# Alxaline/BraTS21

Hardware: AMD Instinct MI355X
Metric: train patches/sec (4x128^3, width-48) (higher is better)
Workload: dtype bf16; 1 GPU; equiunet width=48, batch=2/GPU of 4x128^3 synthetic patches, fwd + deep-supervision Dice + bwd + ranger (BASELINE.json configs[1]); global_batch=2, parallelism=dp1

## Files before the change

### brats21_amd/csrc/dice.hip

```cpp
#include "common.hpp"

__global__ void dice_stats_kernel(const float* __restrict__ x, const float* __restrict__ t, float* __restrict__ part, int K,
                                  size_t voxels) {
  const int nk = blockIdx.y, k = nk % K;
  const float* xp = x + (size_t)nk * voxels;
  const float* tp = t + (size_t)nk * voxels;
  float s0 = 0.f, s1 = 0.f, s2 = 0.f;
  const size_t v4 = (voxels % 4 == 0 && (((size_t)x | (size_t)t) & 15) == 0) ? voxels / 4 : 0;
  for (size_t i = (size_t)blockIdx.x * blockDim.x + threadIdx.x; i < v4; i += (size_t)gridDim.x * blockDim.x) {
    const f32x4 xv = ((const f32x4*)xp)[i], tv = ((const f32x4*)tp)[i];
#pragma unroll
    for (int j = 0; j < 4; ++j) {
      const float p = 1.f / (1.f + __expf(-xv[j]));
      s0 += tv[j] * p;
      s1 += p * p;
      s2 += tv[j] * tv[j];
    }
  }
  for (size_t i = v4 * 4 + (size_t)blockIdx.x * blockDim.x + threadIdx.x; i < voxels; i += (size_t)gridDim.x * blockDim.x) {
    const float p = 1.f / (1.f + __expf(-xp[i]));
    s0 += tp[i] * p; s1 += p * p; s2 += tp[i] * tp[i];
  }
  __shared__ float r[3][256];
  r[0][threadIdx.x] = s0; r[1][threadIdx.x] = s1; r[2][threadIdx.x] = s2;
  __syncthreads();
  for (int m = 128; m > 0; m >>= 1) {
    if ((int)threadIdx.x < m) {
      r[0][threadIdx.x] += r[0][threadIdx.x + m];
      r[1][threadIdx.x] += r[1][threadIdx.x + m];
      r[2][threadIdx.x] += r[2][threadIdx.x + m];
    }
    __syncthreads();
  }
  if (threadIdx.x < 3) part[(((size_t)(nk / K) * gridDim.x + blockIdx.x) * K + k) * 3 + threadIdx.x] = r[threadIdx.x][0];
}

__global__ void __launch_bounds__(256) ordered_sum_kernel(const float* __restrict__ part, float* __restrict__ out, int nb, int total,
                                                          float* __restrict__ out2 , int n1) {
  const int e = threadIdx.x & 7, g = threadIdx.x >> 3;
  const int i = blockIdx.x * 8 + e;
  float s = 0.f;
  if (i < total) {
    const float* src = part + i;
    int b = g;
    for (; b + 7 * 32 < nb; b += 8 * 32) {
      float v[8];
#pragma unroll
      for (int u = 0; u < 8; ++u) v[u] = src[(size_t)(b + 32 * u) * total];
// ... 23 lines not shown
}

__global__ void dice_grad_kernel(const float* __restrict__ x, const float* __restrict__ t, const float* __restrict__ coef,
                                 float* __restrict__ dx, int K, size_t voxels) {
  const int nk = blockIdx.y, k = nk % K;
  const float a = coef[k * 2], b2 = 2.f * coef[k * 2 + 1];
  const float* xp = x + (size_t)nk * voxels;
  const float* tp = t + (size_t)nk * voxels;
  float* dp = dx + (size_t)nk * voxels;
  const size_t v4 = (voxels % 4 == 0 && (((size_t)x | (size_t)t | (size_t)dx) & 15) == 0) ? voxels / 4 : 0;
  for (size_t i = (size_t)blockIdx.x * blockDim.x + threadIdx.x; i < v4; i += (size_t)gridDim.x * blockDim.x) {
    const f32x4 xv = ((const f32x4*)xp)[i], tv = ((const f32x4*)tp)[i];
    f32x4 o;
#pragma unroll
    for (int j = 0; j < 4; ++j) {
      const float p = 1.f / (1.f + __expf(-xv[j]));
      o[j] = (a * tv[j] + b2 * p) * p * (1.f - p);
    }
    ((f32x4*)dp)[i] = o;
  }
  for (size_t i = v4 * 4 + (size_t)blockIdx.x * blockDim.x + threadIdx.x; i < voxels; i += (size_t)gridDim.x * blockDim.x) {
    const float p = 1.f / (1.f + __expf(-xp[i]));
    dp[i] = (a * tp[i] + b2 * p) * p * (1.f - p);
  }
}

constexpr int DICE_MAX_BLOCKS = 512;
extern "C" size_t brats_dice_ws_floats(int N, int K) { return (size_t)N * DICE_MAX_BLOCKS * K * 3; }

extern "C" int brats_dice_stats(const float* logits, const float* target, float* sums , float* ws, int N, int K,
                                size_t voxels, brats_stream_t s) {
  if (!logits || !target || !sums || !ws || N <= 0 || K <= 0) BRATS_FAIL(BRATS_E_ARG, "dice_stats: bad argument");
  hipStream_t st = (hipStream_t)s;
  size_t gx = (voxels / 4 + 255) / 256 / 4;
  gx = gx < 1 ? 1 : (gx > DICE_MAX_BLOCKS ? DICE_MAX_BLOCKS : gx);
  hipLaunchKernelGGL(dice_stats_kernel, dim3((unsigned)gx, N * K), dim3(256), 0, st, logits, target, ws, K, voxels);
  brats_ordered_sum(ws, sums, N * (int)gx, K * 3, st);
  BRATS_CHECK_LAUNCH();
  return 0;
}

extern "C" int brats_dice_grad(const float* logits, const float* target, const float* coef ,
                               float* dlogits, int N, int K, size_t voxels, brats_stream_t s) {
  if (!logits || !target || !coef || !dlogits) BRATS_FAIL(BRATS_E_ARG, "dice_grad: null pointer");
  size_t gx = (voxels / 4 + 255) / 256 / 4;
  gx = gx < 1 ? 1 : (gx > 2048 ? 2048 : gx);
  hipLaunchKernelGGL(dice_grad_kernel, dim3((unsigned)gx, N * K), dim3(256), 0, (hipStream_t)s, logits, target, coef, dlogits, K, voxels);
  BRATS_CHECK_LAUNCH();
  return 0;
}
```

### brats21_amd/csrc/pool_up.hip

```cpp
#include "twin_begin.hpp"
#include "common.hpp"

constexpr int POOL_MAX_BLOCKS = 8192;

template <typename T>
__global__ void maxpool2_fwd_kernel(const T* __restrict__ x, int xpitch, T* __restrict__ y, int ypitch, int N, int C,
                                    int D, int H, int W, int with_avg, uint8_t* __restrict__ argmax) {
  constexpr int VW = 16 / sizeof(T);
  const int cv = C / VW, Do = D / 2, Ho = H / 2, Wo = W / 2;
  const size_t total = (size_t)N * Do * Ho * Wo * cv;
  for (size_t it = (size_t)blockIdx.x * blockDim.x + threadIdx.x; it < total; it += (size_t)gridDim.x * blockDim.x) {
    const int c0 = (int)(it % cv) * VW;
    size_t v = it / cv;
    const int xo = v % Wo; v /= Wo;
    const int yo = v % Ho; v /= Ho;
    const int zo = v % Do;
    const int n = (int)(v / Do);
    float mx[VW], sm[VW];
    int am[VW];
#pragma unroll
    for (int j = 0; j < VW; ++j) { mx[j] = -INFINITY; sm[j] = 0.f; am[j] = 0; }
#pragma unroll
    for (int k = 0; k < 8; ++k) {
      const int z = 2 * zo + (k >> 2), yy = 2 * yo + ((k >> 1) & 1), xx = 2 * xo + (k & 1);
// ... 360 lines not shown
    } else {
      with_stream16(dtype, big, [&](auto t, auto nt) { go(t, nt, std::false_type{}); });
    }
    BRATS_CHECK_LAUNCH();
    return 0;
  }
  with_storage(dtype, [&](auto t) {
    using T = typename decltype(t)::type;
    hipLaunchKernelGGL(upsample_fwd_kernel<T>, dim3(grid), dim3(256), 0, (hipStream_t)s, (const T*)x, xpitch, (T*)y, ypitch, N, C, D, H, W,
                       scale, sd, sh, sw);
  });
  BRATS_CHECK_LAUNCH();
  return 0;
}

template <typename TI, typename TO, int VW>
__global__ void lerp_adjoint_kernel(const TI* __restrict__ in, int in_pitch, TO* __restrict__ out, int out_pitch,
                                    size_t outer, int Lout , int Lin , size_t inner_vox, int C,
                                    float scale) {
  const int cv = C / VW;
  const size_t total = outer * Lin * inner_vox * cv;
  const float inv = scale > 0.f ? 1.f / scale : 0.f;
  for (size_t it = (size_t)blockIdx.x * blockDim.x + threadIdx.x; it < total; it += (size_t)gridDim.x * blockDim.x) {
    const int c0 = (int)(it % cv) * VW;
    size_t v = it / cv;
    const size_t iv = v % inner_vox; v /= inner_vox;
    const int i = (int)(v % Lin);
    const size_t o = v / Lin;
    int lo = (int)floorf((float)(i - 1) * inv) - 1, hi = (int)ceilf((float)(i + 1) * inv) + 1;
    if (scale <= 0.f) { lo = 0; hi = Lout - 1; }
    lo = lo < 0 ? 0 : lo;
    hi = hi > Lout - 1 ? Lout - 1 : hi;
    float acc[VW];
#pragma unroll
    for (int j = 0; j < VW; ++j) acc[j] = 0.f;
    for (int l = lo; l <= hi; ++l) {
      const Lerp c = lerp_coef(l, Lin, scale);
      float w = 0.f;
      if (c.i0 == i) w += c.w0;
      if (c.i1 == i) w += c.w1;
      if (w != 0.f) {
        float a[VW];
        if constexpr (VW == 1) a[0] = to_f<TI>(in[((o * Lout + l) * inner_vox + iv) * in_pitch + c0]);
        else Vec<TI, VW>::load(in + ((o * Lout + l) * inner_vox + iv) * in_pitch + c0, a);
#pragma unroll
        for (int j = 0; j < VW; ++j) acc[j] += w * a[j];
      }
    }
    if constexpr (VW == 1) out[((o * Lin + i) * inner_vox + iv) * out_pitch + c0] = from_f<TO>(acc[0]);
    else Vec<TO, VW>::store(out + ((o * Lin + i) * inner_vox + iv) * out_pitch + c0, acc);
  }
}

int brats_lerp_adjoint_f32_planes(const float* in, float* out, size_t outer, int Lout, int Lin, size_t inner,
                                  hipStream_t st) {
  const size_t total = outer * Lin * inner;
  if (inner % 4 == 0 && (((size_t)in | (size_t)out) & 15) == 0) {
    hipLaunchKernelGGL((lerp_adjoint_kernel<float, float, 4>), dim3(stream_grid(total / 4, 256, POOL_MAX_BLOCKS)), dim3(256), 0, st, in, 4,
                       out, 4, outer, Lout, Lin, inner / 4, 4, ac_scale(Lin, Lout));
    BRATS_CHECK_LAUNCH();
    return 0;
  }
  hipLaunchKernelGGL((lerp_adjoint_kernel<float, float, 1>), dim3(stream_grid(total, 256, POOL_MAX_BLOCKS)), dim3(256), 0, st, in, 1, out, 1,
// ... 18 lines not shown
  float w = 0.f;
  if (c.i0 == i) w += c.w0;
  if (c.i1 == i) w += c.w1;
  return w;
}

constexpr int UBF_TH = 4, UBF_TW = 8, UBF_FH = 12, UBF_FW = 20, UBF_CS = 48, UBF_CV = UBF_CS / 8, UBF_THREADS = 512, UBF_KC = 3, UBF_MAXP = 2;
static_assert(UBF_FH * UBF_FW * UBF_CV <= UBF_THREADS * UBF_KC, "every column of the fine footprint needs a thread slot");
DEVI void ubf_add(float* acc, float w, const bf16_t* p) {
  float a[8];
  Vec<bf16_t, 8>::load(p, a);
#pragma unroll
  for (int j = 0; j < 8; ++j) acc[j] += w * a[j];
}
struct UbfStep { int l[UBF_MAXP]; float wc[UBF_MAXP], wn[UBF_MAXP]; int np; };
__global__ void __launch_bounds__(UBF_THREADS, 4) upsample2_bwd_fused_kernel(const bf16_t* __restrict__ dy, int dypitch, bf16_t* __restrict__ dx,
                                                                          int dxpitch, int C, int D, int H, int W, int cd, float sd,
                                                                          float sh, float sw) {
  __shared__ __attribute__((aligned(16))) bf16_t slab[UBF_FH * UBF_FW * UBF_CS];
  __shared__ __attribute__((aligned(16))) bf16_t t2s[UBF_TH * UBF_FW * UBF_CS];
  __shared__ float wys[UBF_TH][UBF_FH], wxs[UBF_TW][UBF_FW];
  __shared__ int yrng[UBF_TH][2], xrng[UBF_TW][2];
  const int Do = 2 * D, Ho = 2 * H, Wo = 2 * W;
  const int nsl = C / UBF_CS, tiles_x = W / UBF_TW, tiles_y = H / UBF_TH, nz = D / cd;
  int bid = blockIdx.x;
  if (gridDim.x % 8 == 0) bid = (bid % 8) * (gridDim.x / 8) + bid / 8;
  const int sl = bid % nsl, tx = (bid / nsl) % tiles_x, ty = (bid / (nsl * tiles_x)) % tiles_y;
  const int zc = (bid / (nsl * tiles_x * tiles_y)) % nz, n = bid / (nsl * tiles_x * tiles_y * nz);
  const int za = zc * cd, ya = ty * UBF_TH, xa = tx * UBF_TW;
  const int tid = threadIdx.x;
  int yl, yh, xl, xh;
  lerp_fine_range(ya, UBF_TH, H, Ho, sh, yl, yh);
  lerp_fine_range(xa, UBF_TW, W, Wo, sw, xl, xh);
// ... 123 lines not shown
        const float w = wys[h][f];
        if (w != 0.f) ubf_add(acc, w, slab + ((size_t)f * rowv + r) * 8);
      }
      Vec<bf16_t, 8>::store(t2s + (size_t)it * 8, acc);
    }
    __syncthreads();
    for (int it = tid; it < UBF_TH * UBF_TW * UBF_CV; it += UBF_THREADS) {
      const int cvi = it % UBF_CV, xc = (it / UBF_CV) % UBF_TW, h = it / (UBF_CV * UBF_TW);
      float acc[8];
#pragma unroll
      for (int j = 0; j < 8; ++j) acc[j] = 0.f;
      for (int f = xrng[xc][0]; f <= xrng[xc][1]; ++f) {
        const float w = wxs[xc][f];
        if (w != 0.f) ubf_add(acc, w, t2s + ((size_t)(h * fw + f) * UBF_CV + cvi) * 8);
      }
      Vec<bf16_t, 8>::store(dst + (((size_t)i * H + ya + h) * W + xa + xc) * dxpitch + cvi * 8, acc);
    }
  }
}

static int g_upsample_bwd_fused = -1;
extern "C" int BRATS_API(brats_upsample_bwd_set_fused)(int mode) {
  const int old = g_upsample_bwd_fused;
  g_upsample_bwd_fused = mode < 0 ? -1 : (mode ? 1 : 0);
  return old;
}
static int upsample_bwd_fused_cd(int N, int C, int D, int H, int W, int sc) {
  if (g_upsample_bwd_fused == 0 || sc != 2 || C % UBF_CS || H % UBF_TH || W % UBF_TW || D % 4) return 0;
  const size_t per_z = (size_t)N * (H / UBF_TH) * (W / UBF_TW) * (C / UBF_CS);
  int cd = 16;
// ... 124 lines not shown
  else PAF_LAUNCH(6, 2);
#undef PAF_LAUNCH
  BRATS_CHECK_LAUNCH();
  return 0;
}

extern "C" size_t BRATS_API(brats_upsample_bwd_ws_bytes)(int dtype, int N, int C, int D, int H, int W, int scale) {
  const size_t esz = dtype == BRATS_BF16 ? 2 : 4;
  const size_t a = (size_t)N * D * (H * scale) * (W * scale) * C;
  const size_t b = (size_t)N * D * H * (W * scale) * C;
  return ((a * esz + 255) / 256 * 256) + ((b * esz + 255) / 256 * 256);
}

template <typename T>
static int upsample_bwd_t(const T* dy, int dypitch, T* dx, int dxpitch, char* tmp, int N, int C, int D, int H, int W, int sc,
                          hipStream_t st) {
  constexpr int VW = 16 / sizeof(T);
  const int Do = D * sc, Ho = H * sc, Wo = W * sc;
  if constexpr (sizeof(T) == 2) {
    if (const int cd = upsample_bwd_fused_cd(N, C, D, H, W, sc)) {
      const dim3 grid((unsigned)((size_t)N * (H / UBF_TH) * (W / UBF_TW) * (C / UBF_CS) * (D / cd)));
      hipLaunchKernelGGL(upsample2_bwd_fused_kernel, grid, dim3(UBF_THREADS), 0, st, dy, dypitch, dx, dxpitch, C, D, H, W, cd,
                         ac_scale(D, Do), ac_scale(H, Ho), ac_scale(W, Wo));
      BRATS_CHECK_LAUNCH();
      return 0;
    }
  }
  const size_t a_elems = (size_t)N * D * Ho * Wo * C;
  T* t1 = (T*)tmp;
  T* t2 = (T*)(tmp + ((a_elems * sizeof(T) + 255) / 256 * 256));
  size_t total = (size_t)N * D * Ho * Wo * (C / VW);
  hipLaunchKernelGGL((lerp_adjoint_kernel<T, T, VW>), dim3(stream_grid(total, 256, POOL_MAX_BLOCKS)), dim3(256), 0, st, dy, dypitch, t1, C,
                     (size_t)N, Do, D, (size_t)Ho * Wo, C, ac_scale(D, Do));
  total = (size_t)N * D * H * Wo * (C / VW);
  hipLaunchKernelGGL((lerp_adjoint_kernel<T, T, VW>), dim3(stream_grid(total, 256, POOL_MAX_BLOCKS)), dim3(256), 0, st, (const T*)t1, C, t2, C,
                     (size_t)N * D, Ho, H, (size_t)Wo, C, ac_scale(H, Ho));
  total = (size_t)N * D * H * W * (C / VW);
  hipLaunchKernelGGL((lerp_adjoint_kernel<T, T, VW>), dim3(stream_grid(total, 256, POOL_MAX_BLOCKS)), dim3(256), 0, st, (const T*)t2, C, dx,
                     dxpitch, (size_t)N * D * H, Wo, W, (size_t)1, C, ac_scale(W, Wo));
  BRATS_CHECK_LAUNCH();
  return 0;
}

extern "C" int BRATS_API(brats_upsample_bwd)(const void* dy, int dypitch, void* dx, int dxpitch, void* tmp, int dtype, int N, int C,
                                  int D, int H, int W, int scale, brats_stream_t s) {
  const int vw = vec_width(dtype);
  if (!dy || !dx || !tmp || C % vw || dypitch % vw || dxpitch % vw) BRATS_FAIL(BRATS_E_ARG, "upsample_bwd: bad argument");
  return with_storage(dtype, [&](auto t) {
    using T = typename decltype(t)::type;
    return upsample_bwd_t<T>((const T*)dy, dypitch, (T*)dx, dxpitch, (char*)tmp, N, C, D, H, W, scale, (hipStream_t)s);
  });
}
#include "twin_end.hpp"
```

### brats21_amd/engine.py

```python
import torch

from . import ops
from .evaluate import Evaluator
from .optim import clip_grad_norm_
from .losses import DiceLoss, deep_supervision_loss, deep_supervision_prepared_loss, fused_deep_supervision_dice


class TrainStep:

    def __init__(self, model, optimizer, criterion=None, amp=True, buckets=None, fused_dice=True, jaccard=False,
                 max_grad_norm=None, amp_dtype=torch.bfloat16, scaler=None):
        self.model, self.optimizer, self.amp, self.buckets = model, optimizer, amp, buckets
        self.fused, self.jaccard, self.max_grad_norm = fused_dice and criterion is None, jaccard, max_grad_norm
        self.criterion = criterion if criterion is not None else DiceLoss(jaccard=jaccard)
        self.amp_dtype = amp_dtype
        self.scaler = scaler
        self._params = None
        if amp and amp_dtype == torch.float16 and scaler is None:
            self.scaler = torch.amp.GradScaler("cuda")

    def loss(self, outputs, target):
        if self.fused:
            return fused_deep_supervision_dice(outputs, target, jaccard=self.jaccard)
        if hasattr(self.criterion, "prepare"):
            return deep_supervision_prepared_loss(self.criterion, outputs, target)[0]
        return deep_supervision_loss(self.criterion, outputs, target)[0]

    def _zero_grad(self):
        params = self._params
        if params is None:
            params = self._params = list(self.model.parameters())
        for p in params:
# ... 2 lines not shown
    def __call__(self, image, target):
        self._zero_grad()
        with torch.autocast("cuda", dtype=self.amp_dtype, enabled=self.amp):
            outputs = self.model(image)
            loss = self.loss(outputs, target)
        if self.scaler is not None and self.amp:
            self.scaler.scale(loss).backward()
            if self.buckets is not None:
                self.buckets.finish()
            if self.max_grad_norm is not None:
                self.scaler.unscale_(self.optimizer)
                clip_grad_norm_(self._params, self.max_grad_norm)
            self.scaler.step(self.optimizer)
            self.scaler.update()
            return loss
        loss.backward()
        if self.buckets is not None:
            self.buckets.finish()
        if self.max_grad_norm is not None:
            clip_grad_norm_(self._params, self.max_grad_norm)
        self.optimizer.step()
        return loss


class GraphedTrainStep:

    def __init__(self, step, warmup=2, multi_rank_capture=None):
        if getattr(step, "scaler", None) is not None and step.amp:
            if not (getattr(step.optimizer, "_step_supports_amp_scaling", False) and getattr(step.optimizer, "capturable", False)):
                raise NotImplementedError("GraphedTrainStep: a TrainStep with a GradScaler (amp_dtype=torch.float16) captures only with "
                                          "an optimizer that implements the GradScaler protocol on the device "
# ... 55 lines not shown
```

### brats21_amd/losses.py

```python
from collections.abc import Sequence

import torch
import torch.nn as nn


class DiceLoss(nn.Module):
    def __init__(self, jaccard=False, smooth_nr=1e-5, smooth_dr=1e-5):
        super().__init__()
        self.jaccard, self.smooth_nr, self.smooth_dr = jaccard, smooth_nr, smooth_dr

    def forward(self, logits, target):
        p = torch.sigmoid(logits.float())
        t = target.float()
        axes = (0, 2, 3, 4)
        inter = (t * p).sum(axes)
        denom = (t * t).sum(axes) + (p * p).sum(axes)
        if self.jaccard:
            denom = 2.0 * (denom - inter)
        return (1.0 - (2.0 * inter + self.smooth_nr) / (denom + self.smooth_dr)).mean()


def flatten_heads(outputs):
    if isinstance(outputs, (tuple, list)):
        return [h for o in outputs for h in flatten_heads(o)]
    return [outputs]


def deep_supervision_loss(criterion, outputs, target):
    if isinstance(outputs, (tuple, list)):
        heads = flatten_heads(outputs)
        return torch.stack([criterion(h, target) for h in heads]).mean(), heads[0]
    return criterion(outputs, target), outputs


class _FusedDiceFn(torch.autograd.Function):

    @staticmethod
    def forward(ctx, target, jaccard, eps, *heads):
        from . import _lib
        lib = _lib.lib()
        st = torch.cuda.current_stream().cuda_stream
        t = target.contiguous().float()
        n, k = t.shape[:2]
        vox = t[0, 0].numel()
        hs = [h.contiguous().float() for h in heads]
        sums = torch.empty((len(hs), k, 3), dtype=torch.float32, device=t.device)
        ws = torch.empty(lib.brats_dice_ws_floats(n, k), dtype=torch.float32, device=t.device)
        for i, h in enumerate(hs):
            _lib.check(lib.brats_dice_stats(h.data_ptr(), t.data_ptr(), sums[i].data_ptr(), ws.data_ptr(), n, k, vox, st), "dice_stats")
        inter, p2, t2 = sums[..., 0], sums[..., 1], sums[..., 2]
        hk = float(len(hs) * k)
        if jaccard:
            den = 2.0 * (t2 + p2 - inter)
            f = 1.0 - (2.0 * inter + eps) / (den + eps)
            dden = (2.0 * inter + eps) / (den + eps) ** 2
            coef = torch.stack([(-2.0 / (den + eps) - 2.0 * dden) / hk, 2.0 * dden / hk], -1)
        else:
            den = t2 + p2
            f = 1.0 - (2.0 * inter + eps) / (den + eps)
            coef = torch.stack([-2.0 / (den + eps) / hk, (2.0 * inter + eps) / (den + eps) ** 2 / hk], -1)
        ctx.save_for_backward(t, coef.contiguous(), *hs)
        return f.mean()

    @staticmethod
    def backward(ctx, g):
        from . import _lib
        lib = _lib.lib()
        st = torch.cuda.current_stream().cuda_stream
        t, coef, *hs = ctx.saved_tensors
        n, k = t.shape[:2]
        vox = t[0, 0].numel()
        coef = (coef * g).contiguous()
        outs = []
        for i, h in enumerate(hs):
            d = torch.empty_like(h)
            _lib.check(lib.brats_dice_grad(h.data_ptr(), t.data_ptr(), coef[i].data_ptr(), d.data_ptr(), n, k, vox, st), "dice_grad")
            outs.append(d)
        return (None, None, None) + tuple(outs)


def fused_deep_supervision_dice(outputs, target, jaccard=False, eps=1e-5):
    heads = flatten_heads(outputs)
    return _FusedDiceFn.apply(target, jaccard, eps, *heads)


def _check_reference_options(name, sigmoid, softmax, to_onehot_y, other_act, reduction):
# ... 393 lines not shown
```

### brats21_amd/networks/equiunet.py

```python
import contextlib
import functools
import math
import os

import torch
import torch.nn as nn

from .. import ops
from .._lib import PACK_DGRAD, PACK_FWD, BratsHipError
from ._program import _PackedWeightsModule, _fn_backward, _fn_forward, _heads_bwd, _inherit_amax, input_cpad


class _ConvParams(nn.Module):

    def __init__(self, cin, cout, k, bias):
        super().__init__()
        self.weight = nn.Parameter(torch.empty(cout, cin, k, k, k))
        self.bias = nn.Parameter(torch.empty(cout)) if bias else None
        nn.init.kaiming_uniform_(self.weight, a=math.sqrt(5))
        if bias:
            bound = 1.0 / math.sqrt(cin * k * k * k)
            nn.init.uniform_(self.bias, -bound, bound)


# ... 422 lines not shown


def _decoder_bwd(ctx, cx, douts):
    m = cx.m
    _, _, _, _, bottom, bottom_2, up3, up2, up1 = ctx.bufs
    cbw = functools.partial(_cgr_bwd, cx)
    c1, c2 = _blk(m.decoder1)
    top, dsrc = _heads_bwd(ctx, cx, douts, m.fold_head_bwd and cx.drop is None and not c2.batch_norm
                           and ops.head_fold_ok(m.outconv.weight, *_unit_act(c2, cx.act)))

    def extra(t):
        return dsrc.get(t.data_ptr())

    d_c1 = cbw(c2, None, head=top, bst=c1) if top is not None else cbw(c2, extra(up1) if extra(up1) is not None else torch.zeros_like(up1), bst=c1)
    d_skip1, d_u1 = cbw(c1, d_c1)
    d_up2 = _plus(ops.upsample_bwd(d_u1, 2), extra(up2))
    c1, c2 = _blk(m.decoder2)
    d_skip2, d_u2 = cbw(c1, cbw(c2, d_up2, bst=c1))
    d_up3 = _plus(ops.upsample_bwd(d_u2, 2), extra(up3))
    c1, c2 = _blk(m.decoder3)
    d_skip3, d_u3 = cbw(c1, cbw(c2, d_up3, bst=c1))
    return d_skip1, d_skip2, d_skip3, _plus(ops.upsample_bwd(d_u3, 2), extra(bottom_2)), extra(bottom)


class _EquiUnetFn(torch.autograd.Function):
    @staticmethod
    def forward(ctx, model, x, dtype, *params):
        return _fn_forward(_EquiUnetFn._forward, ctx, model, x, dtype, params)

    @staticmethod
    def backward(ctx, *douts):
        return _fn_backward(_EquiUnetFn._backward, ctx, douts)

    @staticmethod
    def _forward(ctx, cx, x0):
        m = cx.m
        cgr = functools.partial(_cgr_fwd, cx)
# ... 89 lines not shown
```

### brats21_amd/ops.py

```python
import contextlib
import weakref

import numpy as np
import torch

from . import _lib
from ._lib import ACT_LEAKY, ACT_NONE, ACT_RELU, BF16, F16, F32, PACK_DGRAD, PACK_FWD, X3_BF16, X3_F16

ACTS = {"none": ACT_NONE, "relu": ACT_RELU, "leakyrelu": ACT_LEAKY, "elu": _lib.ACT_ELU, "swish": _lib.ACT_SWISH,
        "mish": _lib.ACT_MISH}


class KernelTimer:

    def __init__(self):
        self.records = {}

    def span(self, key):
        return _Span(self, key)

    def summary(self):
        torch.cuda.synchronize()
        out = {}
        for key, evs in self.records.items():
# ... 791 lines not shown
def upsample(x, scale=2, out=None):
    ptr, c, p = _desc(x)
    n, d, h, w, _ = x.shape
    if out is None:
        out = new_act(n, d * scale, h * scale, w * scale, c, x.dtype, x.device)
    optr, oc, op = _desc(out)
    _lib.check(_lib.lib().brats_upsample_fwd(ptr, p, optr, op, _code(x.dtype), n, c, d, h, w, scale, _stream()),
               "upsample_fwd")
    return out


def set_upsample_bwd_fused(mode):
    return _lib.lib().brats_upsample_bwd_set_fused(mode)


def upsample_bwd(dy, scale=2):
    dptr, c, dp = _desc(dy)
    n, do, ho, wo, _ = dy.shape
    d, h, w = do // scale, ho // scale, wo // scale
    code = _code(dy.dtype)
    ws = torch.empty(_lib.lib().brats_upsample_bwd_ws_bytes(code, n, c, d, h, w, scale), dtype=torch.uint8, device=dy.device)
    dx = new_act(n, d, h, w, c, dy.dtype, dy.device)
    _lib.check(_lib.lib().brats_upsample_bwd(dptr, dp, dx.data_ptr(), c, ws.data_ptr(), code, n, c, d, h, w, scale,
                                             _stream()), "upsample_bwd")
    return dx


def head(x, weight, bias, scale=1):
    ptr, c, p = _desc(x)
    n, d, h, w, _ = x.shape
    k = weight.shape[0]
    wf = weight.detach().reshape(k, c).contiguous().float()
    out = torch.empty((n, k, d * scale, h * scale, w * scale), dtype=torch.float32, device=x.device)
    low = torch.empty((n, k, d, h, w), dtype=torch.float32, device=x.device) if scale > 1 else None
    _lib.check(_lib.lib().brats_head_fwd(ptr, p, wf.data_ptr(), _f32(bias.detach()) if bias is not None else None,
                                         low.data_ptr() if low is not None else None, out.data_ptr(), _code(x.dtype), n, c,
                                         k, d, h, w, scale, _stream()), "head_fwd")
    return out

# ... 641 lines not shown
```

### include/brats_hip.h

```cpp
#ifndef BRATS_HIP_H
#define BRATS_HIP_H
#include <stddef.h>
#include <stdint.h>

#ifdef __cplusplus
extern "C" {
#endif

typedef void* brats_stream_t;

enum { BRATS_F32 = 0, BRATS_BF16 = 1, BRATS_F16 = 2, BRATS_X3_BF16 = 3, BRATS_X3_F16 = 4 };
enum { BRATS_E_ARG = -1, BRATS_E_UNSUPPORTED = -2, BRATS_E_HIP = -3 };
enum { BRATS_ACT_NONE = 0, BRATS_ACT_RELU = 1, BRATS_ACT_LEAKY = 2, BRATS_ACT_ELU = 3, BRATS_ACT_SWISH = 4, BRATS_ACT_MISH = 5 };

#define BRATS_ABI_VERSION 7
int brats_abi_version(void);
const char* brats_last_error(void);

int brats_dropout(const void* x, int xpitch, void* out, int opitch, int dtype, size_t voxels, int C, float p,
                  const void* state, int unit, brats_stream_t s);

int brats_ncdhw_to_ndhwc(const float* src, void* dst, int dtype, int N, int C, int cpad, int dst_pitch,
                         int D, int H, int W, brats_stream_t s);
int brats_ndhwc_to_ncdhw(const void* src, int src_pitch, float* dst, int dtype, int N, int C,
// ... 173 lines not shown
int brats_maxpool2_fwd(const void* x, int xpitch, void* y, int ypitch,
                       unsigned char* argmax ,
                       int dtype, int N, int C, int D, int H, int W, int with_avg, brats_stream_t s);
int brats_maxpool2_bwd(const void* x, int xpitch, const void* y, int ypitch, const void* dy, int dypitch,
                       const void* dx_skip, int dxskip_pitch, void* dx, int dxpitch, int dtype,
                       int N, int C, int D, int H, int W, int with_avg, brats_stream_t s);
int brats_maxpool2_bwd_idx(const unsigned char* argmax, const void* dy, int dypitch, const void* dx_skip ,
                           int dxskip_pitch, void* dx, int dxpitch, int dtype, int N, int C, int D, int H, int W,
                           int with_avg, brats_stream_t s);

int brats_upsample_fwd(const void* x, int xpitch, void* y, int ypitch, int dtype, int N, int C,
                       int D, int H, int W, int scale, brats_stream_t s);
size_t brats_upsample_bwd_ws_bytes(int dtype, int N, int C, int D, int H, int W, int scale);
int brats_upsample_bwd(const void* dy, int dypitch, void* dx, int dxpitch, void* tmp, int dtype,
                       int N, int C, int D, int H, int W, int scale, brats_stream_t s);
int brats_upsample_bwd_set_fused(int mode);

size_t brats_conv3d_narrow_packed_bytes(int C, int K);
int brats_conv3d_narrow_pack(const float* w, float* packed, int mode, int cout_w, int cin_w, brats_stream_t s);
int brats_conv3d_narrow_fwd(const void* x, int C, int xpitch, const float* packed_w, const float* bias, const float* add, float* out,
                            int dtype, int K, int N, int D, int H, int W, brats_stream_t s);

int brats_head_fwd(const void* x, int xpitch, const float* w , const float* b, float* lowres ,
                   float* out , int dtype, int N, int C, int K,
                   int D, int H, int W, int scale, brats_stream_t s);
int brats_gn_head_fwd(const void* y, int ypitch, const float* scale_shift, int act, float slope, const float* w ,
                      const float* b, float* out, int dtype, int N, int C, int K, int voxels, brats_stream_t s);
int brats_evonorm_head_fwd(const void* y, int ypitch, const float* scale_shift, const float* w , const float* b,
                           float* out, int dtype, int N, int C, int K, int voxels, brats_stream_t s);
size_t brats_head_bwd_ws_bytes(int N, int C, int K, int D, int H, int W, int scale);
// ... 7 lines not shown
                        int Dp, int Hp, int Wp, int rd, int rh, int rw, int n, int z0, int y0, int x0,
                        brats_stream_t s);
int brats_sw_accumulate_multi(const float* prob, const float* importance, float* out, float* count, const int* windows,
                              int B, int NB, int K, int Dp, int Hp, int Wp, int rd, int rh, int rw, brats_stream_t s);
int brats_sw_finalize(const float* out, const float* count, float* dst, int NK, int Dp, int Hp, int Wp,
                      int D, int H, int W, int pad_z, int pad_y, int pad_x, brats_stream_t s);

int brats_spatial_signed_perm(const float* src, float* dst, int planes, int s0, int s1, int s2,
                              int p0, int p1, int p2, int f0, int f1, int f2, int mode, brats_stream_t s);

size_t brats_dice_ws_floats(int N, int K);
int brats_dice_stats(const float* logits, const float* target, float* sums , float* ws, int N, int K,
                     size_t voxels, brats_stream_t s);
int brats_dice_grad(const float* logits, const float* target, const float* coef ,
                    float* dlogits, int N, int K, size_t voxels, brats_stream_t s);

int brats_pad_crop(const float* src, float* dst, int planes, int sd, int sh, int sw, int dd, int dh,
                   int dw, int oz, int oy, int ox, float fill, brats_stream_t s);
int brats_post_threshold(const float* prob, const float* img, float* seg, uint8_t* labels, int N, int K,
                         int C, size_t voxels, float scale, float thresh, brats_stream_t s);
int brats_overlap_counts(const float* pred, const float* target, unsigned long long* counts, int NK,
                         size_t voxels, brats_stream_t s);

size_t brats_cc_ws_bytes(int N, int D, int H, int W);
int brats_cc_filter(uint8_t* labels, int N, int D, int H, int W, int min_size, void* ws, brats_stream_t s);
size_t brats_rare_fill_ws_bytes(int N, int D, int H, int W);
int brats_rare_fill(uint8_t* labels, int N, int D, int H, int W, int axis, int max_count, void* ws,
                    brats_stream_t s);

size_t brats_hausdorff_ws_bytes(int NK, int D, int H, int W);
// ... 149 lines not shown
```

Baseline: 137.5 patches/s.

## Fuse deep-supervision Dice heads into multi-head kernels and fold residual add into upsample backward

Adds multi-head Dice kernels that read the target once and compute stats for all deep-supervision heads in one launch. A single-block finish kernel reduces the partials and computes coefficients and the loss on device. The backward gradient for all heads is also one launch, with the upstream gradient folded in. Separately, upsample backward can now add a stored addend in its epilogue, removing a separate elementwise add in the decoder backward. It also caches the ones tensor passed to loss.backward. The cost is more template instantiations and stricter shape and dtype preconditions; inputs that fail them fall back to the old path.

Measured after the change: 139.8 patches/s (median of 6 runs). 1.02x the previous value.

```diff
diff --git a/brats21_amd/csrc/dice.hip b/brats21_amd/csrc/dice.hip
--- a/brats21_amd/csrc/dice.hip
+++ b/brats21_amd/csrc/dice.hip
@@ -1,4 +1,21 @@
 #include "common.hpp"
+
+DEVI float dice_sigmoid(float x) { return 1.f / (1.f + __expf(-x)); }
+DEVI float dice_grad_elem(float a, float b2, float t, float p) {
+#pragma clang fp contract(off)
+  return (a * t + b2 * p) * p * (1.f - p);
+}
+template <int S>
+DEVI void dice_block_tree(float (*r)[256]) {
+  __syncthreads();
+  for (int m = 128; m > 0; m >>= 1) {
+    if ((int)threadIdx.x < m) {
+#pragma unroll
+      for (int q = 0; q < S; ++q) r[q][threadIdx.x] += r[q][threadIdx.x + m];
+    }
+    __syncthreads();
+  }
+}
 
 __global__ void dice_stats_kernel(const float* __restrict__ x, const float* __restrict__ t, float* __restrict__ part, int K,
                                   size_t voxels) {
@@ -11,27 +28,19 @@
     const f32x4 xv = ((const f32x4*)xp)[i], tv = ((const f32x4*)tp)[i];
 #pragma unroll
     for (int j = 0; j < 4; ++j) {
-      const float p = 1.f / (1.f + __expf(-xv[j]));
+      const float p = dice_sigmoid(xv[j]);
       s0 += tv[j] * p;
       s1 += p * p;
       s2 += tv[j] * tv[j];
     }
   }
   for (size_t i = v4 * 4 + (size_t)blockIdx.x * blockDim.x + threadIdx.x; i < voxels; i += (size_t)gridDim.x * blockDim.x) {
-    const float p = 1.f / (1.f + __expf(-xp[i]));
+    const float p = dice_sigmoid(xp[i]);
     s0 += tp[i] * p; s1 += p * p; s2 += tp[i] * tp[i];
   }
   __shared__ float r[3][256];
   r[0][threadIdx.x] = s0; r[1][threadIdx.x] = s1; r[2][threadIdx.x] = s2;
-  __syncthreads();
-  for (int m = 128; m > 0; m >>= 1) {
-    if ((int)threadIdx.x < m) {
-      r[0][threadIdx.x] += r[0][threadIdx.x + m];
-      r[1][threadIdx.x] += r[1][threadIdx.x + m];
-      r[2][threadIdx.x] += r[2][threadIdx.x + m];
-    }
-    __syncthreads();
-  }
+  dice_block_tree<3>(r);
   if (threadIdx.x < 3) part[(((size_t)(nk / K) * gridDim.x + blockIdx.x) * K + k) * 3 + threadIdx.x] = r[threadIdx.x][0];
 }
 
@@ -85,14 +94,14 @@
     f32x4 o;
 #pragma unroll
     for (int j = 0; j < 4; ++j) {
-      const float p = 1.f / (1.f + __expf(-xv[j]));
-      o[j] = (a * tv[j] + b2 * p) * p * (1.f - p);
+      const float p = dice_sigmoid(xv[j]);
+      o[j] = dice_grad_elem(a, b2, tv[j], p);
     }
     ((f32x4*)dp)[i] = o;
   }
   for (size_t i = v4 * 4 + (size_t)blockIdx.x * blockDim.x + threadIdx.x; i < voxels; i += (size_t)gridDim.x * blockDim.x) {
-    const float p = 1.f / (1.f + __expf(-xp[i]));
-    dp[i] = (a * tp[i] + b2 * p) * p * (1.f - p);
+    const float p = dice_sigmoid(xp[i]);
+    dp[i] = dice_grad_elem(a, b2, tp[i], p);
   }
 }
 
@@ -120,3 +129,241 @@
   BRATS_CHECK_LAUNCH();
   return 0;
 }
+
+constexpr int DICE_MAX_HEADS = 8;
+struct DiceHeadsIn { const float* x[DICE_MAX_HEADS]; };
+struct DiceHeadsOut { float* dx[DICE_MAX_HEADS]; };
+
+template <int H>
+__global__ void __launch_bounds__(256) dice_stats_multi_kernel(DiceHeadsIn hp, const float* __restrict__ t, float* __restrict__ part,
+                                                               size_t head_stride, int K, size_t voxels, int vec_ok) {
+  const int nk = blockIdx.y, k = nk % K;
+  const size_t plane = (size_t)nk * voxels;
+  const float* tp = t + plane;
+  float s0[H], s1[H], s2 = 0.f;
+#pragma unroll
+  for (int h = 0; h < H; ++h) { s0[h] = 0.f; s1[h] = 0.f; }
+  const size_t v4 = vec_ok ? voxels / 4 : 0;
+  for (size_t i = (size_t)blockIdx.x * blockDim.x + threadIdx.x; i < v4; i += (size_t)gridDim.x * blockDim.x) {
+    const f32x4 tv = ((const f32x4*)tp)[i];
+    f32x4 xv[H];
+#pragma unroll
+    for (int h = 0; h < H; ++h) xv[h] = ((const f32x4*)(hp.x[h] + plane))[i];
+#pragma unroll
+    for (int j = 0; j < 4; ++j) {
+#pragma unroll
+      for (int h = 0; h < H; ++h) {
+        const float p = dice_sigmoid(xv[h][j]);
+        s0[h] += tv[j] * p;
+        s1[h] += p * p;
+      }
+      s2 += tv[j] * tv[j];
+    }
+  }
+  for (size_t i = v4 * 4 + (size_t)blockIdx.x * blockDim.x + threadIdx.x; i < voxels; i += (size_t)gridDim.x * blockDim.x) {
+    const float tt = tp[i];
+#pragma unroll
+    for (int h = 0; h < H; ++h) {
+      const float p = dice_sigmoid(hp.x[h][plane + i]);
+      s0[h] += tt * p;
+      s1[h] += p * p;
+    }
+    s2 += tt * tt;
+  }
+  __shared__ float r[2 * H + 1][256];
+#pragma unroll
+  for (int h = 0; h < H; ++h) { r[2 * h][threadIdx.x] = s0[h]; r[2 * h + 1][threadIdx.x] = s1[h]; }
+  r[2 * H][threadIdx.x] = s2;
+  dice_block_tree<2 * H + 1>(r);
+  if (threadIdx.x < 3 * H) {
+    const int h = threadIdx.x / 3, q = threadIdx.x % 3;
+    part[h * head_stride + (((size_t)(nk / K) * gridDim.x + blockIdx.x) * K + k) * 3 + q] = r[q == 2 ? 2 * H : 2 * h + q][0];
+  }
+}
+
+constexpr int DICE_FIN_THREADS = 1024, DICE_MAX_CLASSES = 16;
+DEVI float dice_mean(const float* f, int n, float* tl) {
+#pragma clang fp contract(off)
+  int bw = 1;
+  while (bw * 2 <= n && bw < 64) bw *= 2;
+  for (int j = 0; j < bw; ++j) {
+    float a0 = 0.f, a1 = 0.f, a2 = 0.f, a3 = 0.f;
+    int i = 0;
+    for (int idx = j; idx < n; idx += bw, ++i) {
+      const float v = f[idx];
+      if ((i & 3) == 0) a0 += v;
+      else if ((i & 3) == 1) a1 += v;
+      else if ((i & 3) == 2) a2 += v;
+      else a3 += v;
+    }
+    tl[j] = ((a0 + a1) + a2) + a3;
+  }
+  for (int off = 1; off < bw; off <<= 1)
+    for (int j = 0; j + off < bw; ++j) tl[j] += tl[j + off];
+  return tl[0] * (1.f / (float)n);
+}
+__global__ void __launch_bounds__(DICE_FIN_THREADS) dice_finish_kernel(const float* __restrict__ part, size_t head_stride, int nb, int H, int K,
+                                                                       float eps, int jaccard, float* __restrict__ sums,
+                                                                       float* __restrict__ coef, float* __restrict__ loss) {
+#pragma clang fp contract(off)
+  __shared__ float sm[DICE_FIN_THREADS / 256][32][8];
+  __shared__ float tot[DICE_MAX_HEADS * DICE_MAX_CLASSES * 3], fv[DICE_MAX_HEADS * DICE_MAX_CLASSES];
+  const int K3 = K * 3, total = H * K3;
+  const int c = threadIdx.x >> 8, e = threadIdx.x & 7, g = (threadIdx.x & 255) >> 3;
+  for (int base = 0; base < total; base += DICE_FIN_THREADS / 32) {
+    const int i = base + c * 8 + e;
+    float s = 0.f;
+    if (i < total) {
+      const float* src = part + (size_t)(i / K3) * head_stride + i % K3;
+      int b = g;
+      for (; b + 7 * 32 < nb; b += 8 * 32) {
+        float v[8];
+#pragma unroll
+        for (int u = 0; u < 8; ++u) v[u] = src[(size_t)(b + 32 * u) * K3];
+#pragma unroll
+        for (int u = 0; u < 8; ++u) s += v[u];
+      }
+      for (; b < nb; b += 32) s += src[(size_t)b * K3];
+    }
+    sm[c][g][e] = s;
+    __syncthreads();
+    if (g == 0 && i < total) {
+#pragma unroll
+      for (int k = 1; k < 32; ++k) s += sm[c][k][e];
+      tot[i] = s;
+      sums[i] = s;
+    }
+    __syncthreads();
+  }
+  const int hk = H * K;
+  if ((int)threadIdx.x < hk) {
+    const float inter = tot[threadIdx.x * 3], p2 = tot[threadIdx.x * 3 + 1], t2 = tot[threadIdx.x * 3 + 2];
+    const float inv_hk = 1.f / (float)hk;
+    const float num = 2.f * inter + eps;
+    float c0, c1, de;
+    if (jaccard) {
+      de = 2.f * (t2 + p2 - inter) + eps;
+      const float dden = num / (de * de);
+      c0 = ((1.f / de) * -2.f - 2.f * dden) * inv_hk;
+      c1 = (2.f * dden) * inv_hk;
+    } else {
+      de = t2 + p2 + eps;
+      c0 = ((1.f / de) * -2.f) * inv_hk;
+      c1 = (num / (de * de)) * inv_hk;
+    }
+    coef[threadIdx.x * 2] = c0;
+    coef[threadIdx.x * 2 + 1] = c1;
+    fv[threadIdx.x] = 1.f - num / de;
+  }
+  __syncthreads();
+  if (threadIdx.x == 0) *loss = dice_mean(fv, hk, &sm[0][0][0]);
+}
+
+template <int H>
+__global__ void __launch_bounds__(256) dice_grad_multi_kernel(DiceHeadsIn hp, const float* __restrict__ t, const float* __restrict__ coef,
+                                                              const float* __restrict__ g, DiceHeadsOut op, int K, size_t voxels,
+                                                              int vec_ok) {
+  const int nk = blockIdx.y, k = nk % K;
+  const size_t plane = (size_t)nk * voxels;
+  const float* tp = t + plane;
+  const float up = g[0];
+  float a[H], b2[H];
+#pragma unroll
+  for (int h = 0; h < H; ++h) {
+    a[h] = coef[(h * K + k) * 2] * up;
+    b2[h] = 2.f * (coef[(h * K + k) * 2 + 1] * up);
+  }
+  const size_t v4 = vec_ok ? voxels / 4 : 0;
+  for (size_t i = (size_t)blockIdx.x * blockDim.x + threadIdx.x; i < v4; i += (size_t)gridDim.x * blockDim.x) {
+    const f32x4 tv = ((const f32x4*)tp)[i];
+    f32x4 xv[H];
+#pragma unroll
+    for (int h = 0; h < H; ++h) xv[h] = ((const f32x4*)(hp.x[h] + plane))[i];
+#pragma unroll
+    for (int h = 0; h < H; ++h) {
+      f32x4 o;
+#pragma unroll
+      for (int j = 0; j < 4; ++j) o[j] = dice_grad_elem(a[h], b2[h], tv[j], dice_sigmoid(xv[h][j]));
+      ((f32x4*)(op.dx[h] + plane))[i] = o;
+    }
+  }
+  for (size_t i = v4 * 4 + (size_t)blockIdx.x * blockDim.x + threadIdx.x; i < voxels; i += (size_t)gridDim.x * blockDim.x) {
+    const float tt = tp[i];
+#pragma unroll
+    for (int h = 0; h < H; ++h) op.dx[h][plane + i] = dice_grad_elem(a[h], b2[h], tt, dice_sigmoid(hp.x[h][plane + i]));
+  }
+}
+
+#define DICE_FOR_HEADS(H, CALL) \
+  switch (H) {                  \
+    case 1: { CALL(1); } break; \
+    case 2: { CALL(2); } break; \
+    case 3: { CALL(3); } break; \
+    case 4: { CALL(4); } break; \
+    case 5: { CALL(5); } break; \
+    case 6: { CALL(6); } break; \
+    case 7: { CALL(7); } break; \
+    default: { CALL(8); } break; \
+  }
+
+static size_t dice_stats_blocks(size_t voxels) {
+  const size_t gx = (voxels / 4 + 255) / 256 / 4;
+  return gx < 1 ? 1 : (gx > DICE_MAX_BLOCKS ? DICE_MAX_BLOCKS : gx);
+}
+
+extern "C" size_t brats_dice_multi_ws_floats(int H, int N, int K) { return (size_t)H * brats_dice_ws_floats(N, K); }
+
+extern "C" int brats_dice_stats_multi(const float* const* heads, int H, const float* target, float* ws, int N, int K, size_t voxels,
+                                      brats_stream_t s) {
+  if (!heads || !target || !ws || H < 1 || H > DICE_MAX_HEADS || N <= 0 || K <= 0 || (size_t)N * K > 65535)
+    BRATS_FAIL(BRATS_E_ARG, "dice_stats_multi: bad argument (1 <= heads <= %d)", DICE_MAX_HEADS);
+  DiceHeadsIn hp = {};
+  size_t bits = (size_t)target;
+  for (int h = 0; h < H; ++h) {
+    if (!heads[h]) BRATS_FAIL(BRATS_E_ARG, "dice_stats_multi: null head pointer");
+    hp.x[h] = heads[h];
+    bits |= (size_t)heads[h];
+  }
+  const int vec_ok = voxels % 4 == 0 && (bits & 15) == 0;
+  const dim3 grid((unsigned)dice_stats_blocks(voxels), N * K);
+  const size_t stride = brats_dice_ws_floats(N, K);
+#define DICE_CALL(HH) hipLaunchKernelGGL((dice_stats_multi_kernel<HH>), grid, dim3(256), 0, (hipStream_t)s, hp, target, ws, stride, K, voxels, vec_ok)
+  DICE_FOR_HEADS(H, DICE_CALL)
+#undef DICE_CALL
+  BRATS_CHECK_LAUNCH();
+  return 0;
+}
+
+extern "C" int brats_dice_finish(const float* ws, int H, int N, int K, size_t voxels, float eps, int jaccard, float* sums ,
+                                 float* coef , float* loss, brats_stream_t s) {
+  if (!ws || !sums || !coef || !loss || H < 1 || H > DICE_MAX_HEADS || N <= 0 || K <= 0 || K > DICE_MAX_CLASSES)
+    BRATS_FAIL(BRATS_E_ARG, "dice_finish: bad argument (1 <= heads <= %d, 1 <= classes <= %d)", DICE_MAX_HEADS, DICE_MAX_CLASSES);
+  hipLaunchKernelGGL(dice_finish_kernel, dim3(1), dim3(DICE_FIN_THREADS), 0, (hipStream_t)s, ws, brats_dice_ws_floats(N, K),
+                     N * (int)dice_stats_blocks(voxels), H, K, eps, jaccard, sums, coef, loss);
+  BRATS_CHECK_LAUNCH();
+  return 0;
+}
+
+extern "C" int brats_dice_grad_multi(const float* const* heads, int H, const float* target, const float* coef ,
+                                     const float* g , float* const* dlogits, int N, int K, size_t voxels,
+                                     brats_stream_t s) {
+  if (!heads || !target || !coef || !g || !dlogits || H < 1 || H > DICE_MAX_HEADS || N <= 0 || K <= 0 || (size_t)N * K > 65535)
+    BRATS_FAIL(BRATS_E_ARG, "dice_grad_multi: bad argument (1 <= heads <= %d)", DICE_MAX_HEADS);
+  DiceHeadsIn hp = {};
+  DiceHeadsOut op = {};
+  size_t bits = (size_t)target;
+  for (int h = 0; h < H; ++h) {
+    if (!heads[h] || !dlogits[h]) BRATS_FAIL(BRATS_E_ARG, "dice_grad_multi: null head pointer");
+    hp.x[h] = heads[h];
+    op.dx[h] = dlogits[h];
+    bits |= (size_t)heads[h] | (size_t)dlogits[h];
+  }
+  const int vec_ok = voxels % 4 == 0 && (bits & 15) == 0;
+  size_t gx = (voxels / 4 + 255) / 256 / 4;
+  gx = gx < 1 ? 1 : (gx > 2048 ? 2048 : gx);
+#define DICE_CALL(HH) hipLaunchKernelGGL((dice_grad_multi_kernel<HH>), dim3((unsigned)gx, N * K), dim3(256), 0, (hipStream_t)s, hp, target, coef, g, op, K, voxels, vec_ok)
+  DICE_FOR_HEADS(H, DICE_CALL)
+#undef DICE_CALL
+  BRATS_CHECK_LAUNCH();
+  return 0;
+}
diff --git a/brats21_amd/csrc/pool_up.hip b/brats21_amd/csrc/pool_up.hip
--- a/brats21_amd/csrc/pool_up.hip
+++ b/brats21_amd/csrc/pool_up.hip
@@ -398,10 +398,20 @@
   return 0;
 }
 
-template <typename TI, typename TO, int VW>
+template <typename T, int VW>
+DEVI void add_stored(float* acc, const T* addp) {
+  float b[VW];
+  if constexpr (VW == 1) b[0] = to_f<T>(addp[0]);
+  else Vec<T, VW>::load(addp, b);
+#pragma unroll
+  for (int j = 0; j < VW; ++j) acc[j] = to_f<T>(from_f<T>(acc[j])) + b[j];
+}
+
+template <typename TI, typename TO, int VW, bool ADD = false>
 __global__ void lerp_adjoint_kernel(const TI* __restrict__ in, int in_pitch, TO* __restrict__ out, int out_pitch,
                                     size_t outer, int Lout , int Lin , size_t inner_vox, int C,
-                                    float scale) {
+                                    float scale, const TO* __restrict__ add = nullptr ,
+                                    int add_pitch = 0) {
   const int cv = C / VW;
   const size_t total = outer * Lin * inner_vox * cv;
   const float inv = scale > 0.f ? 1.f / scale : 0.f;
@@ -431,6 +441,7 @@
         for (int j = 0; j < VW; ++j) acc[j] += w * a[j];
       }
     }
+    if constexpr (ADD) add_stored<TO, VW>(acc, add + ((o * Lin + i) * inner_vox + iv) * add_pitch + c0);
     if constexpr (VW == 1) out[((o * Lin + i) * inner_vox + iv) * out_pitch + c0] = from_f<TO>(acc[0]);
     else Vec<TO, VW>::store(out + ((o * Lin + i) * inner_vox + iv) * out_pitch + c0, acc);
   }
@@ -479,9 +490,10 @@
   for (int j = 0; j < 8; ++j) acc[j] += w * a[j];
 }
 struct UbfStep { int l[UBF_MAXP]; float wc[UBF_MAXP], wn[UBF_MAXP]; int np; };
+template <bool ADD>
 __global__ void __launch_bounds__(UBF_THREADS, 4) upsample2_bwd_fused_kernel(const bf16_t* __restrict__ dy, int dypitch, bf16_t* __restrict__ dx,
                                                                           int dxpitch, int C, int D, int H, int W, int cd, float sd,
-                                                                          float sh, float sw) {
+                                                                          float sh, float sw, const bf16_t* __restrict__ add, int addpitch) {
   __shared__ __attribute__((aligned(16))) bf16_t slab[UBF_FH * UBF_FW * UBF_CS];
   __shared__ __attribute__((aligned(16))) bf16_t t2s[UBF_TH * UBF_FW * UBF_CS];
   __shared__ float wys[UBF_TH][UBF_FH], wxs[UBF_TW][UBF_FW];
@@ -635,6 +647,9 @@
         const float w = wxs[xc][f];
         if (w != 0.f) ubf_add(acc, w, t2s + ((size_t)(h * fw + f) * UBF_CV + cvi) * 8);
       }
+      if constexpr (ADD)
+        add_stored<bf16_t, 8>(acc, add + (size_t)n * D * H * W * addpitch + (size_t)sl * UBF_CS +
+                                       (((size_t)i * H + ya + h) * W + xa + xc) * addpitch + cvi * 8);
       Vec<bf16_t, 8>::store(dst + (((size_t)i * H + ya + h) * W + xa + xc) * dxpitch + cvi * 8, acc);
     }
   }
@@ -789,14 +804,18 @@
 
 template <typename T>
 static int upsample_bwd_t(const T* dy, int dypitch, T* dx, int dxpitch, char* tmp, int N, int C, int D, int H, int W, int sc,
-                          hipStream_t st) {
+                          hipStream_t st, const T* add = nullptr, int addpitch = 0) {
   constexpr int VW = 16 / sizeof(T);
   const int Do = D * sc, Ho = H * sc, Wo = W * sc;
   if constexpr (sizeof(T) == 2) {
     if (const int cd = upsample_bwd_fused_cd(N, C, D, H, W, sc)) {
       const dim3 grid((unsigned)((size_t)N * (H / UBF_TH) * (W / UBF_TW) * (C / UBF_CS) * (D / cd)));
-      hipLaunchKernelGGL(upsample2_bwd_fused_kernel, grid, dim3(UBF_THREADS), 0, st, dy, dypitch, dx, dxpitch, C, D, H, W, cd,
-                         ac_scale(D, Do), ac_scale(H, Ho), ac_scale(W, Wo));
+      if (add)
+        hipLaunchKernelGGL(upsample2_bwd_fused_kernel<true>, grid, dim3(UBF_THREADS), 0, st, dy, dypitch, dx, dxpitch, C, D, H, W, cd,
+                           ac_scale(D, Do), ac_scale(H, Ho), ac_scale(W, Wo), add, addpitch);
+      else
+        hipLaunchKernelGGL(upsample2_bwd_fused_kernel<false>, grid, dim3(UBF_THREADS), 0, st, dy, dypitch, dx, dxpitch, C, D, H, W, cd,
+                           ac_scale(D, Do), ac_scale(H, Ho), ac_scale(W, Wo), (const bf16_t*)nullptr, 0);
       BRATS_CHECK_LAUNCH();
       return 0;
     }
@@ -811,8 +830,12 @@
   hipLaunchKernelGGL((lerp_adjoint_kernel<T, T, VW>), dim3(stream_grid(total, 256, POOL_MAX_BLOCKS)), dim3(256), 0, st, (const T*)t1, C, t2, C,
                      (size_t)N * D, Ho, H, (size_t)Wo, C, ac_scale(H, Ho));
   total = (size_t)N * D * H * W * (C / VW);
-  hipLaunchKernelGGL((lerp_adjoint_kernel<T, T, VW>), dim3(stream_grid(total, 256, POOL_MAX_BLOCKS)), dim3(256), 0, st, (const T*)t2, C, dx,
-                     dxpitch, (size_t)N * D * H, Wo, W, (size_t)1, C, ac_scale(W, Wo));
+  if (add)
+    hipLaunchKernelGGL((lerp_adjoint_kernel<T, T, VW, true>), dim3(stream_grid(total, 256, POOL_MAX_BLOCKS)), dim3(256), 0, st, (const T*)t2, C,
+                       dx, dxpitch, (size_t)N * D * H, Wo, W, (size_t)1, C, ac_scale(W, Wo), add, addpitch);
+  else
+    hipLaunchKernelGGL((lerp_adjoint_kernel<T, T, VW>), dim3(stream_grid(total, 256, POOL_MAX_BLOCKS)), dim3(256), 0, st, (const T*)t2, C, dx,
+                       dxpitch, (size_t)N * D * H, Wo, W, (size_t)1, C, ac_scale(W, Wo), (const T*)nullptr, 0);
   BRATS_CHECK_LAUNCH();
   return 0;
 }
@@ -826,4 +849,15 @@
     return upsample_bwd_t<T>((const T*)dy, dypitch, (T*)dx, dxpitch, (char*)tmp, N, C, D, H, W, scale, (hipStream_t)s);
   });
 }
+extern "C" int BRATS_API(brats_upsample_bwd_add)(const void* dy, int dypitch, const void* add, int addpitch, void* dx, int dxpitch,
+                                                 void* tmp, int dtype, int N, int C, int D, int H, int W, int scale, brats_stream_t s) {
+  const int vw = vec_width(dtype);
+  if (!dy || !add || !dx || !tmp || C % vw || dypitch % vw || dxpitch % vw || addpitch % vw)
+    BRATS_FAIL(BRATS_E_ARG, "upsample_bwd_add: bad argument");
+  return with_storage(dtype, [&](auto t) {
+    using T = typename decltype(t)::type;
+    return upsample_bwd_t<T>((const T*)dy, dypitch, (T*)dx, dxpitch, (char*)tmp, N, C, D, H, W, scale, (hipStream_t)s, (const T*)add,
+                             addpitch);
+  });
+}
 #include "twin_end.hpp"
diff --git a/brats21_amd/engine.py b/brats21_amd/engine.py
--- a/brats21_amd/engine.py
+++ b/brats21_amd/engine.py
@@ -16,6 +16,7 @@
         self.amp_dtype = amp_dtype
         self.scaler = scaler
         self._params = None
+        self._one = None
         if amp and amp_dtype == torch.float16 and scaler is None:
             self.scaler = torch.amp.GradScaler("cuda")
 
@@ -48,7 +49,10 @@
             self.scaler.step(self.optimizer)
             self.scaler.update()
             return loss
-        loss.backward()
+        one = self._one
+        if one is None or one.device != loss.device or one.dtype != loss.dtype or one.shape != loss.shape:
+            one = self._one = torch.ones_like(loss, requires_grad=False)
+        loss.backward(one)
         if self.buckets is not None:
             self.buckets.finish()
         if self.max_grad_norm is not None:
diff --git a/brats21_amd/losses.py b/brats21_amd/losses.py
--- a/brats21_amd/losses.py
+++ b/brats21_amd/losses.py
@@ -1,3 +1,4 @@
+import ctypes
 from collections.abc import Sequence
 
 import torch
@@ -33,6 +34,13 @@
     return criterion(outputs, target), outputs
 
 
+MAX_FUSED_HEADS, MAX_FUSED_CLASSES = 8, 16
+
+
+def _pointer_array(tensors):
+    return (ctypes.c_void_p * len(tensors))(*[x.data_ptr() for x in tensors])
+
+
 class _FusedDiceFn(torch.autograd.Function):
 
     @staticmethod
@@ -43,6 +51,20 @@
         t = target.contiguous().float()
         n, k = t.shape[:2]
         vox = t[0, 0].numel()
+        ctx.multi = (len(heads) <= MAX_FUSED_HEADS and k <= MAX_FUSED_CLASSES and n * k <= 65535 and t.is_cuda
+                     and all(h.shape == t.shape and h.dtype == torch.float32 and h.is_contiguous() and h.device == t.device for h in heads))
+        if ctx.multi:
+            nh = len(heads)
+            with torch.cuda.device(t.device):
+                ws = torch.empty(lib.brats_dice_multi_ws_floats(nh, n, k), dtype=torch.float32, device=t.device)
+                sums = torch.empty((nh, k, 3), dtype=torch.float32, device=t.device)
+                coef = torch.empty((nh, k, 2), dtype=torch.float32, device=t.device)
+                loss = torch.empty((), dtype=torch.float32, device=t.device)
+                _lib.check(lib.brats_dice_stats_multi(_pointer_array(heads), nh, t.data_ptr(), ws.data_ptr(), n, k, vox, st), "dice_stats_multi")
+                _lib.check(lib.brats_dice_finish(ws.data_ptr(), nh, n, k, vox, eps, int(bool(jaccard)), sums.data_ptr(), coef.data_ptr(),
+                                                 loss.data_ptr(), st), "dice_finish")
+            ctx.save_for_backward(t, coef, *heads)
+            return loss
         hs = [h.contiguous().float() for h in heads]
         sums = torch.empty((len(hs), k, 3), dtype=torch.float32, device=t.device)
         ws = torch.empty(lib.brats_dice_ws_floats(n, k), dtype=torch.float32, device=t.device)
@@ -70,6 +92,13 @@
         t, coef, *hs = ctx.saved_tensors
         n, k = t.shape[:2]
         vox = t[0, 0].numel()
+        if ctx.multi:
+            g = g.to(device=t.device, dtype=torch.float32)
+            with torch.cuda.device(t.device):
+                outs = [torch.empty_like(h) for h in hs]
+                _lib.check(lib.brats_dice_grad_multi(_pointer_array(hs), len(hs), t.data_ptr(), coef.data_ptr(), g.data_ptr(),
+                                                     _pointer_array(outs), n, k, vox, st), "dice_grad_multi")
+            return (None, None, None) + tuple(outs)
         coef = (coef * g).contiguous()
         outs = []
         for i, h in enumerate(hs):
diff --git a/brats21_amd/networks/equiunet.py b/brats21_amd/networks/equiunet.py
--- a/brats21_amd/networks/equiunet.py
+++ b/brats21_amd/networks/equiunet.py
@@ -460,13 +460,13 @@
 
     d_c1 = cbw(c2, None, head=top, bst=c1) if top is not None else cbw(c2, extra(up1) if extra(up1) is not None else torch.zeros_like(up1), bst=c1)
     d_skip1, d_u1 = cbw(c1, d_c1)
-    d_up2 = _plus(ops.upsample_bwd(d_u1, 2), extra(up2))
+    d_up2 = ops.upsample_bwd(d_u1, 2, add=extra(up2))
     c1, c2 = _blk(m.decoder2)
     d_skip2, d_u2 = cbw(c1, cbw(c2, d_up2, bst=c1))
-    d_up3 = _plus(ops.upsample_bwd(d_u2, 2), extra(up3))
+    d_up3 = ops.upsample_bwd(d_u2, 2, add=extra(up3))
     c1, c2 = _blk(m.decoder3)
     d_skip3, d_u3 = cbw(c1, cbw(c2, d_up3, bst=c1))
-    return d_skip1, d_skip2, d_skip3, _plus(ops.upsample_bwd(d_u3, 2), extra(bottom_2)), extra(bottom)
+    return d_skip1, d_skip2, d_skip3, ops.upsample_bwd(d_u3, 2, add=extra(bottom_2)), extra(bottom)
 
 
 class _EquiUnetFn(torch.autograd.Function):
diff --git a/brats21_amd/ops.py b/brats21_amd/ops.py
--- a/brats21_amd/ops.py
+++ b/brats21_amd/ops.py
@@ -829,15 +829,24 @@
     return _lib.lib().brats_upsample_bwd_set_fused(mode)
 
 
-def upsample_bwd(dy, scale=2):
+def upsample_bwd(dy, scale=2, add=None, out=None):
     dptr, c, dp = _desc(dy)
     n, do, ho, wo, _ = dy.shape
     d, h, w = do // scale, ho // scale, wo // scale
     code = _code(dy.dtype)
     ws = torch.empty(_lib.lib().brats_upsample_bwd_ws_bytes(code, n, c, d, h, w, scale), dtype=torch.uint8, device=dy.device)
-    dx = new_act(n, d, h, w, c, dy.dtype, dy.device)
-    _lib.check(_lib.lib().brats_upsample_bwd(dptr, dp, dx.data_ptr(), c, ws.data_ptr(), code, n, c, d, h, w, scale,
-                                             _stream()), "upsample_bwd")
+    dx = new_act(n, d, h, w, c, dy.dtype, dy.device) if out is None else out
+    xptr, xc, xp = _desc(dx)
+    if tuple(dx.shape) != (n, d, h, w, c) or dx.dtype != dy.dtype:
+        raise ValueError(f"upsample_bwd: out {tuple(dx.shape)} {dx.dtype} does not match {(n, d, h, w, c)} {dy.dtype}")
+    if add is None:
+        _lib.check(_lib.lib().brats_upsample_bwd(dptr, dp, xptr, xp, ws.data_ptr(), code, n, c, d, h, w, scale, _stream()), "upsample_bwd")
+        return dx
+    if tuple(add.shape) != (n, d, h, w, c) or add.dtype != dy.dtype:
+        raise ValueError(f"upsample_bwd: addend {tuple(add.shape)} {add.dtype} does not match {(n, d, h, w, c)} {dy.dtype}")
+    aptr, _, ap = _desc(add)
+    _lib.check(_lib.lib().brats_upsample_bwd_add(dptr, dp, aptr, ap, xptr, xp, ws.data_ptr(), code, n, c, d, h, w, scale, _stream()),
+               "upsample_bwd_add")
     return dx
 
 
diff --git a/include/brats_hip.h b/include/brats_hip.h
--- a/include/brats_hip.h
+++ b/include/brats_hip.h
@@ -211,6 +211,8 @@
 size_t brats_upsample_bwd_ws_bytes(int dtype, int N, int C, int D, int H, int W, int scale);
 int brats_upsample_bwd(const void* dy, int dypitch, void* dx, int dxpitch, void* tmp, int dtype,
                        int N, int C, int D, int H, int W, int scale, brats_stream_t s);
+int brats_upsample_bwd_add(const void* dy, int dypitch, const void* add, int addpitch, void* dx, int dxpitch, void* tmp,
+                           int dtype, int N, int C, int D, int H, int W, int scale, brats_stream_t s);
 int brats_upsample_bwd_set_fused(int mode);
 
 size_t brats_conv3d_narrow_packed_bytes(int C, int K);
@@ -248,6 +250,13 @@
                      size_t voxels, brats_stream_t s);
 int brats_dice_grad(const float* logits, const float* target, const float* coef ,
                     float* dlogits, int N, int K, size_t voxels, brats_stream_t s);
+size_t brats_dice_multi_ws_floats(int H, int N, int K);
+int brats_dice_stats_multi(const float* const* heads, int H, const float* target, float* ws, int N, int K, size_t voxels,
+                           brats_stream_t s);
+int brats_dice_finish(const float* ws, int H, int N, int K, size_t voxels, float eps, int jaccard, float* sums, float* coef,
+                      float* loss, brats_stream_t s);
+int brats_dice_grad_multi(const float* const* heads, int H, const float* target, const float* coef, const float* g,
+                          float* const* dlogits, int N, int K, size_t voxels, brats_stream_t s);
 
 int brats_pad_crop(const float* src, float* dst, int planes, int sd, int sh, int sw, int dd, int dh,
                    int dw, int oz, int oy, int ox, float fill, brats_stream_t s);
```
